# yanconglin/ICP-Flow

Measured on AMD Instinct MI355X. Metric: cluster-pair ICP registrations/sec, higher is better.
Workload: dtype f32

## Files before the change

### icp_flow_amd/build.py

```python
import argparse
import concurrent.futures
import hashlib
import os
import subprocess
import sys

HERE = os.path.dirname(os.path.abspath(__file__))
CSRC = os.path.join(HERE, "csrc")
OBJ = os.path.join(CSRC, "_obj")
OUT = os.path.join(HERE, "libicpflow_hip.so")
SOURCES = ["api.hip", "hist.hip", "nn.hip", "icp.hip", "icp_prep.hip", "icp_plan.hip", "icp_epilogue.hip", "device.hip", "icp_fp32.hip", "pose.hip", "sort.hip", "cluster.hip", "hdbscan.hip", "clusterpcd.hip", "table.hip", "assoc.hip", "frame.hip", "ego.hip", "seqeval.hip", "classeval.hip", "bucketeval.hip", "segeval.hip", "ground.hip", "nnresid.hip", "segresid.hip", "sight.hip",
           "hdbscan_tree.cpp"]
HEADERS = ["common.hpp", "scan.hpp", "kernels.hpp", "kabsch.hpp", "posefuse.hpp", "votekey.hpp", "cluster_util.hpp", "sortdir.hpp", "sortclouds.hpp", "occgrid.hpp", "host.hpp", "carver.hpp", "rowerr.hpp", "clusterpcd_host.hpp", "gridhash.hpp", "nnresid.hpp", "sight.hpp", "icp_instr.hip",
           os.path.join("..", "..", "include", "icpflow_hip.h")]
CFLAGS = ["--offload-arch=gfx950", "-O3", "-std=c++17", "-fPIC", "-ffp-contract=off",
          "-fhip-fp32-correctly-rounded-divide-sqrt", "-Wall", "-Wno-unused-function"]


def hipcc():
    for c in (os.environ.get("HIPCC"), "/opt/rocm/bin/hipcc", "hipcc"):
        if c and (os.path.isabs(c) and os.path.exists(c) or not os.path.isabs(c)):
            return c
    return "hipcc"


def _digest(paths, extra=()):
    h = hashlib.sha256()
    for p in paths:
        h.update(os.path.basename(p).encode())
        with open(p, "rb") as f:
            h.update(f.read())
    for e in extra:
        h.update(str(e).encode())
    return h.hexdigest()


# ... 87 lines not shown
```

### icp_flow_amd/csrc/api.hip

```cpp
#include <stdarg.h>
#include <stdio.h>
#include <stdlib.h>
#include <string.h>

#include "kernels.hpp"
#include "posefuse.hpp"
#include "kabsch.hpp"
#include "host.hpp"

using namespace icpflow;

namespace {

thread_local char g_err[512] = "";

}

namespace icpflow {
int report_error(int code, const char *message)
{
    snprintf(g_err, sizeof(g_err), "%s", message);
    return code;
}

// ... 322 lines not shown
    int dev = -1;
    if (hipGetDevice(&dev) != hipSuccess) { none.ok = false; return none; }
    for (int k = 0; k < kSlots; ++k)
        if (slots[k].used && slots[k].caller == caller && slots[k].s.device == dev) return slots[k].s;
    Slot &sl = slots[next];
    next = (next + 1) % kSlots;
    if (!sl.used || sl.s.device != dev) {
        sl.s.destroy();
        sl.s = SideStream{};
        sl.s.create();
    }
    sl.used = true;
    sl.caller = caller;
    return sl.s;
}

struct JoinGuard {
    hipStream_t s = nullptr;
    hipEvent_t join = nullptr;
    ~JoinGuard() { if (join != nullptr) (void)hipStreamWaitEvent(s, join, 0); }
    void joined() { join = nullptr; }
};

int run_icp_and_select(const float *src, const float *dst, Workspace &w, const uint8_t *swap,
                       const float *init, int B, int N, double thres, int maxIter, double relThr,
                       int stopMode, int invertSwapped, float *Tout, int32_t *iters, const Opts &o, hipStream_t s,
                       bool teamPlanned = false, int part = 0, int32_t *pending = nullptr, bool initSumValid = false)
{
    const GridScratch *search = search_scratch(w, N, o);
    const bool sweepCheck = search != nullptr && search->mode == 3 && o.on(ICPFLOW_OPT_NO_CHECK_SWEEP);
    bool historyPending = false;
    IcpOpts io = o.icp(w.grid.sortX);
    io.help = icp_help_carve(w.ctrl, B, w.helpState, w.helpOut);
    io.splitScratch = w.icpSplit;
    io.teamPlanned = teamPlanned;
    if (sweepCheck && o.arith == ICPFLOW_ARITH_FP64) io.historyPending = &historyPending;
    const bool splittable = sweepCheck && o.arith == ICPFLOW_ARITH_FP64 && stopMode == ICPFLOW_STOP_REFERENCE && w.history != nullptr &&
                            o.on(ICPFLOW_OPT_NO_SPECULATIVE) && maxIter > 1 && maxIter <= kHistIters;
    if (part == 1) {
        *pending = 0;
        if (!splittable) return 0;
        if (icp_teams_wanted(&w.team, io, search, B, N, maxIter, stopMode, w.history)) return 0;
        io.pairActive = nullptr;
    }
    if (part == 2 && pending != nullptr && *pending != 0) {
        historyPending = true;
        if (o.pairActive != nullptr) ICPFLOW_TRY(launch_icp_retally(w.ctrl, w.history, o.pairActive, B, maxIter, relThr, s));
    } else {
        ICPFLOW_TRY(launch_icp(src, dst, w.lenA, w.lenC, swap, init, B, N, thres, maxIter, relThr, stopMode,
                               w.state, w.ctrl, search, w.history, &w.team, io, s));
        if (part == 1) {
            if (!historyPending) return report_errorf(ICPFLOW_E_ARG, "icpflow_register_stage_begin: the ICP launch kept no history");
            *pending = 1;
            return 0;
        }
    }
    if (sweepCheck) {
        PoseSource ps{w.state, w.ctrl, historyPending ? w.history : nullptr, init, B, maxIter};
        const double *initSum = (initSumValid && search->presorted && o.on(ICPFLOW_OPT_NO_CHECK_REUSE)) ? w.scoreAccum : nullptr;
        ICPFLOW_TRY(launch_sweep_check(search, src, dst, w.lenA, w.lenC, swap, B, N, init, nullptr, w.partial, s, &ps, o.pairActive,
                                       initSum));
        ICPFLOW_TRY(launch_select(w.partial, sweep_qblocks(N), w.lenA, w.lenC, swap, init, nullptr, B, invertSwapped,
                                  Tout, s, &ps, iters, initSum, o.pairActive));
        return 0;
    }
    ICPFLOW_TRY(launch_compose(w.state, init, B, w.M, s, w.ctrl, iters));
    {
        ICPFLOW_TRY(launch_scan_check(src, dst, w.lenA, w.lenC, swap, B, N, init, w.M, w.partial, s));
        ICPFLOW_TRY(launch_select(w.partial, scan_qblocks(N, B), w.lenA, w.lenC, swap, init, w.M, B,
                                  invertSwapped, Tout, s));
    }
    return 0;
}

int run_init_pose(const float *src, const float *dst, Workspace &w, const uint8_t *swap, int B,
                  int N, const float *ex, int lx, const float *ey, int ly, const float *ez, int lz,
                  float shift, float *Tout, const Opts &o, hipStream_t s, hipEvent_t joinBefore = nullptr,
                  const PairCountFuse *countFuse = nullptr, bool sideBusy = false, const FrontRoles *roles = nullptr)
{
    const int lens[3] = {lx, ly, lz};
    if (N <= kMaxSortN && o.on(ICPFLOW_OPT_NO_SORTED_VOTE)) {
        bool planned = false;
        ICPFLOW_TRY(launch_hist_vote_sorted(dst, src, w.lenC, w.lenA, B, N, lens, ex, ey, ez, swap, w.zsortC,
                                            w.zsortA, w.bins, w.zckey, w.zcidx, w.voteKey, s, countFuse, sideBusy,
                                            w.grid.pairBox, o.on(ICPFLOW_OPT_NO_VOTE_LIST) ? w.voteWork : nullptr, w.voteWorkCap,
                                            w.pairOrder, &planned, roles));
        if (planned) w.grid.pairOrder = w.pairOrder;
    } else
        ICPFLOW_TRY(launch_hist_vote(dst, src, B, N, N, nullptr, nullptr, lens, ex, ey, ez, swap, w.bins, s));
    if (o.voteBins != nullptr)
        ICPFLOW_TRY(hipMemcpyAsync(o.voteBins, w.bins, (size_t)B * lx * ly * lz * sizeof(uint32_t),
                                   hipMemcpyDeviceToDevice, s));
    if (w.pairTab != nullptr && B <= 700 && N <= kMaxSortN && o.on(ICPFLOW_OPT_NO_SORTED_VOTE)) {
        ICPFLOW_TRY(launch_sweep_pair_table(w.lenA, w.lenC, swap, w.grid.pairOrder, B, N, w.pairTab, s));
        w.grid.pairTab = w.pairTab;
    }
    PeakDecode dec;
    dec.ex = ex; dec.ey = ey; dec.ez = ez; dec.shift = shift; dec.cand = w.cand;
    ICPFLOW_TRY(launch_hist_peaks_u32(w.bins, B, lx, ly, lz, kTopK, kNmsKernel, w.volA, w.volB,
                                      w.peakVotes, w.peakIdx, s, dec));
    if (score_by_sweep(N, joinBefore != nullptr || w.grid.presorted, o)) {
        if (joinBefore != nullptr) {
            ICPFLOW_TRY(hipStreamWaitEvent(s, joinBefore, 0));
        } else if (!w.grid.presorted) {
            ICPFLOW_TRY(launch_sort_clouds_soa(src, dst, w.lenA, w.lenC, swap, B, N, &w.grid, s));
            w.grid.presorted = 1;
            if (o.on(ICPFLOW_OPT_NO_SCORE_PRUNE) && o.on(ICPFLOW_OPT_NO_SCORE_PREBOUND)) {
                ICPFLOW_TRY(launch_occupancy(&w.grid, B, N, s));
                w.grid.occReady = 1;
            }
        }
        if (o.on(ICPFLOW_OPT_NO_SCORE_PRUNE))
            ICPFLOW_TRY(launch_sweep_score_pruned(&w.grid, w.lenA, w.lenC, swap, B, N, w.cand, w.partial, w.scoreAccum, s));
        else
            ICPFLOW_TRY(launch_sweep_score(&w.grid, w.lenA, w.lenC, swap, B, N, w.cand, w.partial, s));
        ICPFLOW_TRY(launch_score_pick(w.partial, sweep_qblocks(N), w.lenA, w.lenC, swap, w.cand, B, Tout, s, w.scoreAccum));
        w.initSumValid = true;
    } else if (o.on(ICPFLOW_OPT_NO_SCORE_PRUNE)) {
        ICPFLOW_TRY(launch_scan_score_pruned(src, dst, w.lenA, w.lenC, swap, B, N, w.cand, w.partial, w.scoreAccum, s, true));
        ICPFLOW_TRY(launch_score_pick(w.partial, score_qblocks(N), w.lenA, w.lenC, swap, w.cand, B, Tout, s));
    } else {
        ICPFLOW_TRY(launch_scan_score(src, dst, w.lenA, w.lenC, swap, B, N, w.cand, w.partial, s));
        ICPFLOW_TRY(launch_score_pick(w.partial, scan_qblocks(N, B), w.lenA, w.lenC, swap, w.cand, B, Tout, s));
    }
    return 0;
}

}

extern "C" {

int icpflow_version(void) { return ICPFLOW_VERSION; }

#ifndef ICPFLOW_SOURCE_HASH
#define ICPFLOW_SOURCE_HASH "unknown"
#endif
static const char g_build_info[] = "ICPFLOW_SOURCE_HASH=" ICPFLOW_SOURCE_HASH;
const char *icpflow_build_info(void) { return g_build_info + sizeof("ICPFLOW_SOURCE_HASH=") - 1; }

const char *icpflow_last_error(void) { return g_err; }
// ... 576 lines not shown
            if (se == hipSuccess) w.grid.occReady = 1;
        }
        if (se == hipSuccess && !countInSort && phase != 1 &&
            icp_teams_wanted(&w.team, o.icp(w.grid.sortX), search, B, N, max_iterations, stop_mode, w.history)) {
            launch_icp_team_plan(&w.team, w.lenA, w.lenC, w.swap, B, N, o.icp(w.grid.sortX), side->stream);
            teamPlanned = true;
        }
        const hipError_t je = hipEventRecord(side->join, side->stream);
        if (je == hipSuccess) { guard.s = s; guard.join = side->join; }
        ICPFLOW_TRY(se);
        ICPFLOW_TRY(je);
        w.grid.presorted = 1;
        join = side->join;
    }
    PairCountFuse fuse{};
    if (countInSort) {
        fuse.swapOut = w.swap;
        fuse.zero0 = w.ctrl; fuse.bytes0 = icp_ctrl_bytes(B);
        fuse.zero1 = w.scoreAccum; fuse.bytes1 = w.accumBytes;
    }
    w.grid.shareCountClean = 1;
    w.grid.sweepTicket = w.ticketScratch;
    const bool sweepScore = score_by_sweep(N, join != nullptr || frontRoles, o);
    if (int r = run_init_pose(d_src, d_dst, w, w.swap, B, N, d_edges_x, len_x, d_edges_y, len_y, d_edges_z,
                              len_z, decode_shift, w.Tinit, o, s, sweepScore ? join : nullptr,
                              countInSort ? &fuse : nullptr, join != nullptr, frontRoles ? &roles : nullptr))
        return r;
    if (join != nullptr && !sweepScore) ICPFLOW_TRY(hipStreamWaitEvent(s, join, 0));
    guard.joined();
    if (phase == 1) {
        carry[0] = w.grid.presorted;
        carry[1] = teamPlanned ? 1 : 0;
        carry[3] = w.initSumValid ? 1 : 0;
        return run_icp_and_select(d_src, d_dst, w, w.swap, w.Tinit, B, N, thres_dist, max_iterations, relative_rmse_thr,
                                  stop_mode, 1, d_T_out, d_iters, o, s, teamPlanned, 1, &carry[2]);
    }
    return run_icp_and_select(d_src, d_dst, w, w.swap, w.Tinit, B, N, thres_dist, max_iterations,
                              relative_rmse_thr, stop_mode, 1, d_T_out, d_iters, o, s, teamPlanned, 0, nullptr, w.initSumValid);
}

int icpflow_hist_icp(const float *d_src, const float *d_dst, int B, int N, const float *d_edges_x,
                     int len_x, const float *d_edges_y, int len_y, const float *d_edges_z, int len_z,
                     float decode_shift, double thres_dist, int max_iterations, double relative_rmse_thr,
                     int stop_mode, float *d_T_out, int32_t *d_iters, void *d_ws, size_t ws_bytes,
                     icpflow_stream_t stream, const icpflow_options_t *opt)
{
    Opts o;
    if (int r = parse_options("icpflow_hist_icp", opt, o)) return r;
    if (int r = check_arith("icpflow_hist_icp", o, max_iterations, stop_mode)) return r;
    if (int r = check_pair_active("icpflow_hist_icp", o, true, max_iterations, stop_mode)) return r;
    if (!d_src || !d_dst || !d_edges_x || !d_edges_y || !d_edges_z || !d_T_out)
        return report_errorf(ICPFLOW_E_ARG, "icpflow_hist_icp: null pointer");
    if (int r = check_batch("icpflow_hist_icp", B, N)) return r;
    if (int r = check_hist_dims("icpflow_hist_icp", len_x, len_y, len_z)) return r;
    if (max_iterations <= 0 || max_iterations > kMaxIterCap)
        return report_errorf(ICPFLOW_E_ARG, "icpflow_hist_icp: max_iterations must be in 1..%d", kMaxIterCap);
    if (stop_mode != ICPFLOW_STOP_REFERENCE && stop_mode != ICPFLOW_STOP_PER_PAIR)
        return report_errorf(ICPFLOW_E_ARG, "icpflow_hist_icp: unknown stop_mode %d", stop_mode);
    const size_t L = (size_t)len_x * len_y * len_z;
    if (L < (size_t)kTopK) return report_errorf(ICPFLOW_E_ARG, "icpflow_hist_icp: fewer than 5 bins");
    Workspace w(d_ws, B, N, L);
// ... 181 lines not shown
```

### icp_flow_amd/csrc/icp.hip

```cpp
#include <atomic>
#include <mutex>

#include "scan.hpp"
#include "sortdir.hpp"
#include "kernels.hpp"
#include "gridhash.hpp"
#include "icp_instr.hip"
#include "kabsch.hpp"

namespace icpflow {

struct IcpParams {
#ifdef ICPFLOW_CERT_STATS
    const float *occHdr;
    const uint32_t *occBits;
#endif
    const float *X;
    const float *Y;
    const int32_t *lenX;
    const int32_t *lenY;
    const uint8_t *swap;
    const float *prePose;
    int N;
    float thr2;
    float relThr;
    int stopMode;
    int maxIter;
    IcpState *state;
    IcpCtrl *ctrl;
    const float4 *gridPts;
    const int32_t *gridStart;
// ... 9 lines not shown
    float *history;
    int B;
    IcpTeam team;
    const float *initR;
    const float *initT;
    int allowReflection;
    int estimateScale;
    const float *initS;
    int halfCu;
    int persistent;
    IcpHelp help;
    int helpOn;
    int redPasses;
    int x0Cache;
    int recCap;
    int shareScans;
    int teamLanes;
    const uint8_t *pairActive;
    int drainAt;
    const int32_t *pairList;
    const int32_t *pairMeta;
    int twoLaunch;
    int32_t *splitScratch;
};


constexpr int kMoments = 18;

__device__ __forceinline__ int state_hash_word(float w, int k)
{
    const unsigned u = (unsigned)__float_as_int(w);
    return (int)__builtin_amdgcn_alignbit(u, u, (unsigned)((5 * k + 3) & 31));
}
constexpr int kRecMaxN = 4096;
#ifndef ICPFLOW_PROBE_MAX
#define ICPFLOW_PROBE_MAX 20
#endif
constexpr int kProbeMax = ICPFLOW_PROBE_MAX;
#ifndef ICPFLOW_PROBE_STEPS
#define ICPFLOW_PROBE_STEPS 8
#endif
constexpr int kProbeSteps = ICPFLOW_PROBE_STEPS;
#ifndef ICPFLOW_PROBE_MAX_LONG
#define ICPFLOW_PROBE_MAX_LONG 32
#endif
#ifndef ICPFLOW_PROBE_STEPS_LONG
// ... 100 lines not shown
#ifdef ICPFLOW_NO_SHARE
    constexpr bool SHARE = false;
#else
    constexpr bool SHARE = SHAREK && TEAM && GRID == 4 && Q == 1;
#endif
    __shared__ int shHdr[SHARE ? NWAVE : 1][4];
    __shared__ int shNext[SHARE ? NWAVE : 1], shDone[SHARE ? NWAVE : 1], shLock[SHARE ? NWAVE : 1];
    __shared__ unsigned int shAcc[SHARE ? NWAVE : 1][3][kWave];
    __shared__ unsigned int shState;
    [[maybe_unused]] const bool helping = HELP && role != 0;
    [[maybe_unused]] HelpPair *hp = nullptr;
    if constexpr (HELP) hp = (p.helpOn && p.help.pair != nullptr) ? p.help.pair + b : nullptr;
    IcpTeam team{};
    if constexpr (TEAM) {
        team.wgPair = p.team.wgPair; team.wgRank = p.team.wgRank; team.teamSize = p.team.teamSize;
        team.arrived = p.team.arrived; team.mom = p.team.mom; team.maxWG = p.team.maxWG;
    }
    const int tid = threadIdx.x;
    const int lane = tid & (kWave - 1);
    const int wave = tid >> 6;
    const int ts = wave % TS;
    const int qg = wave / TS;
    IcpCtrl *ctrl = p.ctrl;
    if (p.pairActive != nullptr && p.history != nullptr && p.pairActive[b] == 0) {
        if (rank == 0 && wave == 0)
            for (int k = itBegin + lane; k < p.maxIter; k += kWave)
                __hip_atomic_fetch_add(&ctrl->tally[k], 1ull, __ATOMIC_RELAXED, __HIP_MEMORY_SCOPE_AGENT);
        if (tid == 0 && rank == 0) {
            IcpState *st0 = p.state + b;
#pragma unroll
            for (int k = 0; k < 9; ++k) st0->R[k] = (k % 4 == 0) ? 1.f : 0.f;
            st0->T[0] = st0->T[1] = st0->T[2] = 0.f;
            st0->rmse = 0.f; st0->s = 1.f; st0->active = 0; st0->iters = 0;
            if constexpr (HELP) {
                if (p.drainAt > 0) __hip_atomic_fetch_add(&ctrl->finished, 1, __ATOMIC_RELAXED, __HIP_MEMORY_SCOPE_AGENT);
            }
        }
        return;
    }
    if (p.stopMode == ICPFLOW_STOP_REFERENCE_ && itBegin > 0 && p.history == nullptr) {
        if (ctrl->done || ctrl->notconv[itBegin - 1] == 0) {
            if (tid == 0 && b == 0) ctrl->done = 1;
            return;
        }
    }
    const bool sw = p.swap != nullptr && p.swap[b] != 0;
    CloudView xc, yc;
    xc.base = (sw ? p.Y : p.X) + (size_t)b * p.N * 4; xc.stride = 4; xc.n = (sw ? p.lenY : p.lenX)[b];
    yc.base = (sw ? p.X : p.Y) + (size_t)b * p.N * 4; yc.stride = 4; yc.n = (sw ? p.lenX : p.lenY)[b];
    PointXf pre;
    pre.kind = p.prePose ? XF_AFFINE : XF_NONE;
    pre.a = p.prePose ? affine_from_pose(p.prePose + (size_t)b * 16) : affine_identity();
    PointXf none;
    none.kind = XF_NONE;
    none.a = affine_identity();

    IcpState *st = p.state + b;
    int active = 1;
    constexpr bool RESUME = BLOCK == 1024 && GRID == 4 && !TEAM && !SCALE && !HELP && LATE && Q == 1 && WIDE;
    const bool resumed = RESUME && itBegin > 0 && p.history != nullptr;
    if (itBegin == 0 || (resumed && itBegin < kRing)) {
        float s0 = (tid < 9 && tid % 4 == 0) ? 1.f : 0.f;
        if (p.initR != nullptr && tid < 12) s0 = tid < 9 ? p.initR[(size_t)b * 9 + tid] : p.initT[(size_t)b * 3 + tid - 9];
        const float scale0 = p.initS != nullptr ? p.initS[b] : 1.f;
        if (itBegin == 0) {
            if (tid < 12) bcast[tid] = s0;
            if (tid == 0) { bcast[12] = 1.f; bcast[13] = 0.f; bcast[14] = 0.f; bcast[15] = scale0; }
        }
        if (tid < 16) ring[tid] = tid < 12 ? s0 : (tid == 14 ? scale0 : 0.f);
        if (tid < kWave) {
            int hash = 0;
#pragma unroll
            for (int k = 0; k < 12; ++k) hash ^= state_hash_word(__shfl(s0, k, kWave), k);
            hash ^= state_hash_word(scale0, 12);
            if (tid == 13) ring[13] = __int_as_float(hash);
// ... 18 lines not shown
                    if (on) ring[(n % kRing) * 16 + w] = w == 13 ? __int_as_float(hw) : hv;
                }
            }
        }
    }
    int itersDone = (itBegin == 0) ? 0 : st->iters;
    if (tid == 0) { probeCnt[0] = 0; probeCnt[1] = 0; probeNext[0] = 0; probeNext[1] = 0; }
    if (SHARE && tid == 0) shState = 0u;
    [[maybe_unused]] int hbSeq = 0;
    [[maybe_unused]] int probePar = 0;

    if (tid == 0) {
        float o0 = 0.f, o1 = 0.f, o2 = 0.f;
        if (xc.n > 0) {
            float rx, ry, rz;
            cloud_load(xc, 0, rx, ry, rz);
            xf_apply(pre, rx, ry, rz, o0, o1, o2);
        }
        bcast[16] = o0; bcast[17] = o1; bcast[18] = o2;
#pragma unroll
        for (int k = 0; k < 9; ++k) preL[k] = pre.a.m[k];
#pragma unroll
        for (int k = 0; k < 3; ++k) preL[9 + k] = pre.a.t[k];
    }
    __syncthreads();

    const int per = NQG * kWave * Q;
    const int ngroups = (xc.n + per - 1) / per;

    int itFirst = itBegin;
    if constexpr (HELP) {
        if (tid == 0) helpSh[0] = 0;
        if (hp == nullptr) __syncthreads();
        if (hp != nullptr && !helping) {
            if (tid == 0) {
                __hip_atomic_store(&hp->passes, (xc.n + BLOCK - 1) / BLOCK, __ATOMIC_RELAXED, __HIP_MEMORY_SCOPE_AGENT);
                __hip_atomic_store(&hp->iter, itBegin + 1, __ATOMIC_RELAXED, __HIP_MEMORY_SCOPE_AGENT);
                __hip_atomic_store(&p.help.owner[blockIdx.x], b + 1, __ATOMIC_RELAXED, __HIP_MEMORY_SCOPE_AGENT);
            }
            __syncthreads();
        }
        if (helping) {
            if (tid == 0) {
                int e = 0;
                const int cur = __hip_atomic_load(&hp->iter, __ATOMIC_RELAXED, __HIP_MEMORY_SCOPE_AGENT);
                if (cur > 0) {
// ... 118 lines not shown
            const int NP16 = (p.N + kChunk - 1) / kChunk * kChunk;
            const int np16 = (yc.n + kChunk - 1) / kChunk * kChunk;
            const float *gx = p.sortYsoa + (size_t)b * 3 * NP16;
            const float *gy = gx + NP16;
            const float *gz = gy + NP16;
            const float4 *ys = p.sortY + (size_t)b * p.N;
            const float4 *xs = p.sortX + (size_t)b * p.N;
            const int axis = sweepAxis;
            float dirX = 0.f, dirY = 0.f;
            if (WIDE && axis >= 3) sort_dir(axis, dirX, dirY);
            unsigned char *dyn = dynLds + (size_t)p.redPasses * (NWAVE * kMoments * sizeof(double));
            float *lx = reinterpret_cast<float *>(dyn), *ly = lx + NP16, *lz = ly + NP16;
            const bool perPass = !TEAM && WIDE && p.redPasses != 0;
            double *redDyn = reinterpret_cast<double *>(dynLds);
            constexpr bool REC = (GRID == 4);
            const int unitsAll = (xc.n + kWave - 1) / kWave;
            const bool dealt = TEAM && G > 1;
            const int myCount = dealt ? (unitsAll > rank ? (unitsAll - rank + G - 1) / G : 0) * kWave : xc.n;
            float4 *rec = reinterpret_cast<float4 *>(dyn + (size_t)NP16 * 12);
            int *recJ = reinterpret_cast<int *>(dyn + (size_t)NP16 * 12 + (size_t)p.recCap * 16);
            const bool recOn = REC && p.recCap > 0 && myCount <= p.recCap;
            float *x0c = reinterpret_cast<float *>(dyn + (size_t)NP16 * 12 + (size_t)p.recCap * 20);
            const bool x0On = recOn && p.x0Cache != 0;
            if (GRID == 4 && it == itFirst) {
                for (int k = tid; k < np16; k += BLOCK) { lx[k] = gx[k]; ly[k] = gy[k]; lz[k] = gz[k]; }
                __syncthreads();
            }
            const float *keyf = (GRID == 4) ? (axis == 0 ? lx : (axis == 1 ? ly : lz))
                                            : (axis == 0 ? gx : (axis == 1 ? gy : gz));
            auto tkey = [&](int j) -> float {
                return (WIDE && axis >= 3) ? sort_key_dir(dirX, dirY, (GRID == 4 ? lx : gx)[j], (GRID == 4 ? ly : gy)[j]) : keyf[j];
            };
            auto pkey = [&](float x, float y, float z) -> float {
                if constexpr (WIDE) return sort_key_of(axis, dirX, dirY, x, y, z);
                else return axis == 0 ? x : (axis == 1 ? y : z);
            };
            auto keySlack = [&](float x, float y, float r) -> float { return WIDE ? sort_key_slack(axis, x, y, r) : 0.f; };
            constexpr int PER = BLOCK * Q;
            const int ngr = (myCount + PER - 1) / PER;
            double fold[5] = {0.0, 0.0, 0.0, 0.0, 0.0};
            bool reuseMoments = false;
            [[maybe_unused]] int helpedPasses = 0;
            if constexpr (HELP) helpedPasses = helping ? 0 : __builtin_amdgcn_readfirstlane(helpSh[0]);
            [[maybe_unused]] bool shareOn = false;
            if constexpr (SHARE) shareOn = recOn && p.shareScans != 0 && yc.n >= kShareMinN;
            [[maybe_unused]] auto unit_query = [&](int gp, int uw, float &ux, float &uy, float &uz) {
                const int li = gp * PER + uw * kWave + lane;
// ... 1409 lines not shown
    } else if (p.gridPts != nullptr) {
        if (p.N <= 256) launch_icp_variant<256, 1, 1, 2>(p, B, itBegin, itEnd, s);
        else if (p.N <= 2048) launch_icp_variant<1024, 1, 1, 2>(p, B, itBegin, itEnd, s);
        else launch_icp_variant<1024, 1, 1, 1>(p, B, itBegin, itEnd, s);
    } else {
        if (p.N <= 256) launch_icp_variant<256, 2, 2, 0>(p, B, itBegin, itEnd, s);
        else if (p.N <= 512) launch_icp_variant<512, 2, 2, 0>(p, B, itBegin, itEnd, s);
        else if (p.N <= 1024) launch_icp_variant<1024, 4, 4, 0>(p, B, itBegin, itEnd, s);
        else launch_icp_variant<1024, 4, 2, 0>(p, B, itBegin, itEnd, s);
    }
    if (timed) profile_stop(prof, s);
}

bool icp_teams_wanted(const IcpTeam *team, const IcpOpts &opts, const GridScratch *grid, int B, int N, int maxIter,
                      int stopMode, const float *history)
{
    const bool speculative = stopMode == ICPFLOW_STOP_REFERENCE_ && history != nullptr && opts.speculative &&
                             maxIter > 1 && maxIter <= kHistIters;
    return opts.arith != ICPFLOW_ARITH_FP32_REFERENCE && team != nullptr && opts.teams && grid != nullptr && grid->mode == 3 &&
           N > 1024 && 2 * B <= device_cus() && B <= 256 && B <= min(icp_team_workgroups(opts), team->maxWG) &&
           (speculative || stopMode == ICPFLOW_STOP_PER_PAIR_);
}

hipError_t launch_icp(const float *X, const float *Y, const int32_t *lenX, const int32_t *lenY,
                      const uint8_t *swap, const float *prePose, int B, int N, double thres,
                      int maxIter, double relThr, int stopMode, IcpState *state, IcpCtrl *ctrl,
                      const GridScratch *grid, float *history, const IcpTeam *team, const IcpOpts &opts,
                      hipStream_t s)
{
    if (opts.arith == ICPFLOW_ARITH_FP32_REFERENCE) {
        if (history == nullptr || opts.fp32Scratch == nullptr || maxIter > kHistIters ||
            stopMode != ICPFLOW_STOP_REFERENCE_)
            return hipErrorInvalidValue;
        return launch_icp_fp32ref(X, Y, lenX, lenY, swap, prePose, B, N, thres, maxIter, relThr, state, ctrl, history,
                                  opts.fp32Scratch, s);
    }
    IcpParams p{};
    bool dirKeys = true;
    p.B = B;
    p.X = X; p.Y = Y; p.lenX = lenX; p.lenY = lenY; p.swap = swap; p.prePose = prePose; p.N = N;
    p.thr2 = (float)(thres * thres);
    p.relThr = (float)relThr;
    p.stopMode = stopMode; p.maxIter = maxIter; p.state = state; p.ctrl = ctrl;
    p.initR = opts.initR; p.initT = opts.initT; p.allowReflection = opts.allowReflection ? 1 : 0;
    p.initS = opts.initS; p.estimateScale = opts.estimateScale ? 1 : 0;
    hipError_t e = hipSuccess;
    bool recWanted = false;
    if (opts.historyPending != nullptr) *opts.historyPending = false;
    if (!opts.ctrlCleared) {
        e = hipMemsetAsync(ctrl, 0, icp_ctrl_bytes(B), s);
        if (e != hipSuccess) return e;
    }
// ... 1 lines not shown
        p.sortX = (const float4 *)grid->sortX; p.sortY = (const float4 *)grid->pts; p.sortAxis = grid->axis;
        dirKeys = N >= kSortDirMinN;
        p.sortYsoa = grid->sortYsoa;
        p.sweepMargin = (float)(1.01 * thres);
#ifdef ICPFLOW_CERT_STATS
        if (grid->occReady) { p.occHdr = grid->occHdr; p.occBits = grid->occBits; }
#endif
        p.sortedRaw = 1;
        recWanted = opts.adaptiveWindows;
    } else if (grid != nullptr && grid->mode == 3) {
        e = launch_sort_clouds(X, Y, lenX, lenY, swap, prePose, B, N, grid, false, nullptr, 0, s);
        if (e != hipSuccess) return e;
        p.sortX = (const float4 *)grid->sortX; p.sortY = (const float4 *)grid->pts; p.sortAxis = grid->axis;
        dirKeys = grid->dirKeys && N >= kSortDirMinN;
        p.sortYsoa = grid->sortYsoa;
        p.sweepMargin = (float)(1.01 * thres);
        recWanted = opts.adaptiveWindows;
    } else if (grid != nullptr) {
        const float invh = (float)(1.0 / (1.01 * thres));
        launch_grid_build(X, Y, lenX, lenY, swap, B, N, invh, grid, s);
        p.gridPts = (const float4 *)grid->pts; p.gridStart = grid->start; p.gridOrigin = grid->origin;
        p.gridH = grid->H; p.gridInvH = invh;
    }
    const int cus = device_cus();
    const bool speculative = stopMode == ICPFLOW_STOP_REFERENCE_ && history != nullptr && opts.speculative &&
                             maxIter > 1 && maxIter <= kHistIters;
    if (icp_teams_wanted(team, opts, grid, B, N, maxIter, stopMode, history)) {
        p.team = *team;
        p.team.maxWG = min(icp_team_workgroups(opts), team->maxWG);
        p.teamLanes = opts.teamsHalfGpu ? 2 : 1;
        if (!opts.teamPlanned) launch_icp_team_plan(team, lenX, lenY, swap, B, N, opts, s);
    }
    if (p.sortY != nullptr) {
        const size_t img = (size_t)((N + kChunk - 1) / kChunk * kChunk) * 12;
        const size_t room = p.team.wgPair != nullptr ? icp_team_room(opts, N) : (size_t)152 * 1024;
        int recCap = 0;
        if (p.team.wgPair != nullptr) {
            if (N <= 12288 && img + 64 * 20 <= room) recCap = (int)((room - img) / 20 / 64 * 64);
            p.shareScans = (recWanted && recCap > 0 && icp_team_shares(opts, N)) ? 1 : 0;
        } else if (N <= kRecMaxN) {
            recCap = N;
        }
        bool x0Cache = recCap > 0 && img + (size_t)recCap * 32 <= room;
        const size_t half = 76 * 1024;
#ifndef ICPFLOW_HALF_CU_MIN_N
#define ICPFLOW_HALF_CU_MIN_N 768
#endif
        const double fillHalf = (double)B / ((double)((B + 2 * cus - 1) / (2 * cus)) * 2 * cus);
        const double fillFull = (double)B / ((double)((B + cus - 1) / cus) * cus);
        const size_t redHalf = N <= kRecMaxN ? (size_t)((N + 511) / 512) * 8 * kMoments * sizeof(double) : 0;
        const size_t redFull = N <= kRecMaxN ? (size_t)((N + 1023) / 1024) * 16 * kMoments * sizeof(double) : 0;
        if (p.team.wgPair == nullptr && B >= 2 * cus && N > ICPFLOW_HALF_CU_MIN_N && redHalf + img + (size_t)recCap * 20 <= half &&
            1.1 * fillHalf > fillFull) {
            p.halfCu = 1;
            x0Cache = redHalf + img + (size_t)recCap * 32 <= half;
        } else if (p.team.wgPair == nullptr) {
            x0Cache = x0Cache && redFull + img + (size_t)recCap * 32 <= room;
        }
        if (recWanted) { p.recCap = recCap; p.x0Cache = x0Cache ? 1 : 0; }
    }
    if (stopMode == ICPFLOW_STOP_REFERENCE_) {
        if (speculative) {
            p.history = history;
            p.pairActive = opts.pairActive;
            p.persistent = opts.persistent ? 1 : 0;
            p.twoLaunch = (opts.twoLaunch && opts.splitScratch != nullptr) ? 1 : 0;
            p.splitScratch = opts.splitScratch;
            p.help = opts.help;
            p.helpOn = (opts.helpers && maxIter <= kHelpMaxEpoch - 2) ? 1 : 0;
            launch_icp_iters(p, dirKeys, B, 0, maxIter, opts.profile, s);
            if (opts.historyPending != nullptr) {
                *opts.historyPending = true;
            } else {
                e = launch_icp_resolve_history(state, ctrl, history, B, maxIter, s);
                if (e != hipSuccess) return e;
            }
        } else {
            for (int it = 0; it < maxIter; ++it) launch_icp_iters(p, dirKeys, B, it, it + 1, opts.profile, s);
        }
    } else {
        p.persistent = opts.persistent ? 1 : 0;
        p.help = opts.help;
        p.helpOn = (opts.helpers && maxIter <= kHelpMaxEpoch - 2) ? 1 : 0;
        launch_icp_iters(p, dirKeys, B, 0, maxIter, opts.profile, s);
    }
    return hipGetLastError();
}

}
```

### icp_flow_amd/csrc/kernels.hpp

```cpp
#pragma once
#include <hip/hip_runtime.h>
#include <atomic>
#include <stddef.h>
#include <stdint.h>

#include "../../include/icpflow_hip.h"

namespace icpflow {

constexpr int ICPFLOW_STOP_REFERENCE_ = ICPFLOW_STOP_REFERENCE;
constexpr int ICPFLOW_STOP_PER_PAIR_ = ICPFLOW_STOP_PER_PAIR;

constexpr int kPartial = 8;
constexpr int kMaxIterCap = 1024;
constexpr int kCand = 6;
constexpr int kTopK = 5;
constexpr int kNmsKernel = 11;

struct IcpState {
    float R[9];
    float T[3];
    float rmse;
    int active;
    int iters;
// ... 169 lines not shown
    int32_t *cursor;
    float *pts;
    float *sortX;
    float *sortYsoa;
    float *sortXsoa;
    int32_t *axis;
    int dirKeys;
    float *ckey;
    int *cidx;
    const float *pairBox;
    const int32_t *pairTab;
    const int32_t *pairOrder;
    float *shareBest;
    int *shareCount;
    int shareCountClean;
    float *occHdr;
    uint32_t *occBits;
    int occReady;
    int32_t *occTot;
    int *sweepTicket;
    int *scoreList;
    int presorted;
};
struct LaunchProfile;
struct IcpOpts {
    int arith = 0;
    bool teams = true;
    bool speculative = true;
    bool adaptiveWindows = true;
    bool persistent = true;
    bool helpers = true;
    IcpHelp help{};
    const float *initR = nullptr;
    const float *initT = nullptr;
    bool allowReflection = false;
    bool estimateScale = false;
    const float *initS = nullptr;
    LaunchProfile *profile = nullptr;
    bool ctrlCleared = false;
    bool *historyPending = nullptr;
    float *fp32Scratch = nullptr;
    bool teamPlanned = false;
    const uint8_t *pairActive = nullptr;
    bool teamsHalfGpu = false;
    bool sharedScans = true;
    bool twoLaunch = false;
    int32_t *splitScratch = nullptr;
};

int device_cus();
void ensure_dynamic_lds(const void *func, int bytes, std::atomic<unsigned long long> *doneMask);
LaunchProfile *profile_create(int capacity, hipError_t *err);
void profile_destroy(LaunchProfile *p);
hipError_t profile_collect(LaunchProfile *p, double *total_ms, int *launches);
bool profile_start(LaunchProfile *p, hipStream_t s);
void profile_stop(LaunchProfile *p, hipStream_t s);

int grid_buckets(int N);
void launch_grid_build(const float *X, const float *Y, const int32_t *lenX, const int32_t *lenY, const uint8_t *swap, int B,
                       int N, float invh, const GridScratch *grid, hipStream_t s);
hipError_t launch_sort_clouds(const float *X, const float *Y, const int32_t *lenX, const int32_t *lenY, const uint8_t *swap,
                              const float *prePose, int B, int N, const GridScratch *grid, bool wantXsoa, const float *boxes,
                              int selfCount, hipStream_t s);
hipError_t launch_sort_clouds_soa(const float *X, const float *Y, const int32_t *lenX, const int32_t *lenY,
                                  const uint8_t *swap, int B, int N, const GridScratch *grid, hipStream_t s, int selfCount = 0);

int icp_team_workgroups(const IcpOpts &opts);
bool icp_team_shares(const IcpOpts &opts, int N);
size_t icp_team_room(const IcpOpts &opts, int N);
void launch_icp_team_plan(const IcpTeam *team, const int32_t *lenX, const int32_t *lenY, const uint8_t *swap, int B, int N,
                          const IcpOpts &opts, hipStream_t s);

bool icp_teams_wanted(const IcpTeam *team, const IcpOpts &opts, const GridScratch *grid, int B, int N, int maxIter,
                      int stopMode, const float *history);
hipError_t launch_icp(const float *X, const float *Y, const int32_t *lenX, const int32_t *lenY,
                      const uint8_t *swap, const float *prePose, int B, int N, double thres,
                      int maxIter, double relThr, int stopMode, IcpState *state, IcpCtrl *ctrl,
                      const GridScratch *grid, float *history, const IcpTeam *team, const IcpOpts &opts,
                      hipStream_t s);
hipError_t launch_icp_fp32ref(const float *X, const float *Y, const int32_t *lenX, const int32_t *lenY,
                              const uint8_t *swap, const float *prePose, int B, int N, double thres, int maxIter,
                              double relThr, IcpState *state, IcpCtrl *ctrl, float *history, float *nnScratch,
                              hipStream_t s);

hipError_t launch_icp_resolve_history(IcpState *state, IcpCtrl *ctrl, const float *history, int B, int maxIter,
                                      hipStream_t s);
hipError_t launch_icp_export(IcpState *state, IcpCtrl *ctrl, int B, int stopMode, float *R,
                             float *T, float *rmse, int32_t *iters, int32_t *converged, hipStream_t s,
                             float *scale = nullptr);
void launch_icp_split(const IcpCtrl *ctrl, const IcpState *state, int B, int maxIter, int32_t *list, int32_t *meta, hipStream_t s);
hipError_t launch_icp_retally(IcpCtrl *ctrl, const float *history, const uint8_t *active, int B, int maxIter, double relThr,
                              hipStream_t s);

hipError_t launch_score_pick(const double *partial, int qblocks, const int32_t *lenA,
                             const int32_t *lenC, const uint8_t *swap, const float *cand, int B,
                             float *Tinit, hipStream_t s, double *initSum = nullptr);
hipError_t launch_compose(const IcpState *state, const float *init, int B, float *M, hipStream_t s,
// ... 62 lines not shown
```

### icp_flow_amd/csrc/pose.hip

```cpp
#include "common.hpp"
#include "kernels.hpp"
#include "posefuse.hpp"

namespace icpflow {

__device__ __forceinline__ double partial_total(const double *partial, int job, int qblocks, int k)
{
    double s = 0.0;
    const double *base = partial + (size_t)job * qblocks * kPartial + k;
    if (qblocks <= 4) {
        double v[4];
#pragma unroll
        for (int u = 0; u < 4; ++u) v[u] = base[(size_t)min(u, qblocks - 1) * kPartial];
#pragma unroll
        for (int u = 0; u < 4; ++u)
            if (u < qblocks) s += v[u];
        return s;
    }
    for (int q0 = 0; q0 < qblocks; q0 += 8) {
        double v[8];
#pragma unroll
        for (int u = 0; u < 8; ++u) v[u] = base[(size_t)min(q0 + u, qblocks - 1) * kPartial];
#pragma unroll
        for (int u = 0; u < 8; ++u)
            if (q0 + u < qblocks) s += v[u];
    }
    return s;
}

__global__ __launch_bounds__(kWave) void score_pick_kernel(const double *__restrict__ partial, int qblocks,
                                                           const int32_t *__restrict__ lenA,
                                                           const int32_t *__restrict__ lenC,
                                                           const uint8_t *__restrict__ swap,
                                                           const float *__restrict__ cand, int B,
                                                           float *__restrict__ Tinit, double *__restrict__ initSum)
{
    const int b = blockIdx.x, lane = threadIdx.x;
    const bool sw = swap != nullptr && swap[b] != 0;
    const float na = (float)(sw ? lenC[b] : lenA[b]);
    const float nc = (float)(sw ? lenA[b] : lenC[b]);
    float mean = 0.f;
    double total = 0.0;
    if (lane < 2 * kCand) {
        total = partial_total(partial, b * 12 + lane, qblocks, 0);
        mean = (float)total / ((lane & 1) ? nc : na);
    }
    int pick = 0;
    float best = 0.f;
    for (int k = 0; k < kCand; ++k) {
        const float sc = fminf(__shfl(mean, 2 * k, kWave), __shfl(mean, 2 * k + 1, kWave));
        if (k == 0 || sc < best) { best = sc; pick = k; }
    }
    if (initSum != nullptr && lane == 2 * pick) initSum[b] = total;
    if (lane < 16) {
        const float *t = cand + ((size_t)b * kCand + pick) * 3;
        float v = (lane % 5 == 0) ? 1.f : 0.f;
        if (lane == 3) v = t[0];
        if (lane == 7) v = t[1];
        if (lane == 11) v = t[2];
        Tinit[(size_t)b * 16 + lane] = v;
    }
}

hipError_t launch_score_pick(const double *partial, int qblocks, const int32_t *lenA,
                             const int32_t *lenC, const uint8_t *swap, const float *cand, int B,
                             float *Tinit, hipStream_t s, double *initSum)
{
    hipLaunchKernelGGL(score_pick_kernel, dim3(B), dim3(kWave), 0, s, partial, qblocks, lenA, lenC, swap, cand, B,
                       Tinit, initSum);
    return hipGetLastError();
}

__global__ void compose_kernel(const IcpState *__restrict__ st, const float *__restrict__ init, int B,
                               float *__restrict__ M, const IcpCtrl *__restrict__ ctrl, int32_t *__restrict__ iters)
{
    const int b = blockIdx.x * blockDim.x + threadIdx.x;
    if (b == 0 && iters != nullptr) *iters = ctrl->error ? -1 : ctrl->iters;
    if (b >= B) return;
    float A[16];
    for (int i = 0; i < 3; ++i) {
        for (int j = 0; j < 3; ++j) A[i * 4 + j] = st[b].R[j * 3 + i];
        A[i * 4 + 3] = st[b].T[i];
    }
    A[12] = A[13] = A[14] = 0.f; A[15] = 1.f;
// ... 340 lines not shown
```

Before: 439,700.

## Fuse candidate score pick into the ICP kernel prologue

Moves the per-pair score-pick step, which chooses the best initial translation candidate, into the first wave of the ICP kernel, so the separate score_pick launch is skipped whenever the speculative grid-mode ICP path qualifies. While wave 0 picks, the other waves preload the sorted target SoA into LDS in the prologue instead of at the first iteration. The goal is to remove one kernel launch and its dependency gap per batch. The cost is a more complex eligibility check that must agree between host and kernel, plus some extra prologue work in the ICP kernel.

```diff
diff --git a/icp_flow_amd/build.py b/icp_flow_amd/build.py
--- a/icp_flow_amd/build.py
+++ b/icp_flow_amd/build.py
@@ -11,7 +11,7 @@
 OUT = os.path.join(HERE, "libicpflow_hip.so")
 SOURCES = ["api.hip", "hist.hip", "nn.hip", "icp.hip", "icp_prep.hip", "icp_plan.hip", "icp_epilogue.hip", "device.hip", "icp_fp32.hip", "pose.hip", "sort.hip", "cluster.hip", "hdbscan.hip", "clusterpcd.hip", "table.hip", "assoc.hip", "frame.hip", "ego.hip", "seqeval.hip", "classeval.hip", "bucketeval.hip", "segeval.hip", "ground.hip", "nnresid.hip", "segresid.hip", "sight.hip",
            "hdbscan_tree.cpp"]
-HEADERS = ["common.hpp", "scan.hpp", "kernels.hpp", "kabsch.hpp", "posefuse.hpp", "votekey.hpp", "cluster_util.hpp", "sortdir.hpp", "sortclouds.hpp", "occgrid.hpp", "host.hpp", "carver.hpp", "rowerr.hpp", "clusterpcd_host.hpp", "gridhash.hpp", "nnresid.hpp", "sight.hpp", "icp_instr.hip",
+HEADERS = ["common.hpp", "scan.hpp", "kernels.hpp", "kabsch.hpp", "posefuse.hpp", "scorepick.hpp", "votekey.hpp", "cluster_util.hpp", "sortdir.hpp", "sortclouds.hpp", "occgrid.hpp", "host.hpp", "carver.hpp", "rowerr.hpp", "clusterpcd_host.hpp", "gridhash.hpp", "nnresid.hpp", "sight.hpp", "icp_instr.hip",
            os.path.join("..", "..", "include", "icpflow_hip.h")]
 CFLAGS = ["--offload-arch=gfx950", "-O3", "-std=c++17", "-fPIC", "-ffp-contract=off",
           "-fhip-fp32-correctly-rounded-divide-sqrt", "-Wall", "-Wno-unused-function"]
diff --git a/icp_flow_amd/csrc/api.hip b/icp_flow_amd/csrc/api.hip
--- a/icp_flow_amd/csrc/api.hip
+++ b/icp_flow_amd/csrc/api.hip
@@ -368,10 +368,29 @@
     void joined() { join = nullptr; }
 };
 
+static bool icp_splittable(const Workspace &w, const GridScratch *search, const Opts &o, int stopMode, int maxIter)
+{
+    const bool sweepCheck = search != nullptr && search->mode == 3 && o.on(ICPFLOW_OPT_NO_CHECK_SWEEP);
+    return sweepCheck && o.arith == ICPFLOW_ARITH_FP64 && stopMode == ICPFLOW_STOP_REFERENCE && w.history != nullptr &&
+           o.on(ICPFLOW_OPT_NO_SPECULATIVE) && maxIter > 1 && maxIter <= kHistIters;
+}
+
+static bool pick_in_icp(Workspace &w, const Opts &o, int B, int N, int maxIter, int stopMode, int phase, bool sweepScore)
+{
+    if (!sweepScore || phase == 2) return false;
+    const GridScratch *search = search_scratch(w, N, o);
+    const IcpOpts io = o.icp(w.grid.sortX);
+    if (phase == 1 && (!icp_splittable(w, search, o, stopMode, maxIter) ||
+                       icp_teams_wanted(&w.team, io, search, B, N, maxIter, stopMode, w.history)))
+        return false;
+    return icp_pick_in_icp(&w.team, io, search, true, B, N, maxIter, stopMode, w.history);
+}
+
 int run_icp_and_select(const float *src, const float *dst, Workspace &w, const uint8_t *swap,
                        const float *init, int B, int N, double thres, int maxIter, double relThr,
                        int stopMode, int invertSwapped, float *Tout, int32_t *iters, const Opts &o, hipStream_t s,
-                       bool teamPlanned = false, int part = 0, int32_t *pending = nullptr, bool initSumValid = false)
+                       bool teamPlanned = false, int part = 0, int32_t *pending = nullptr, bool initSumValid = false,
+                       bool pickInIcp = false)
 {
     const GridScratch *search = search_scratch(w, N, o);
     const bool sweepCheck = search != nullptr && search->mode == 3 && o.on(ICPFLOW_OPT_NO_CHECK_SWEEP);
@@ -381,8 +400,7 @@
     io.splitScratch = w.icpSplit;
     io.teamPlanned = teamPlanned;
     if (sweepCheck && o.arith == ICPFLOW_ARITH_FP64) io.historyPending = &historyPending;
-    const bool splittable = sweepCheck && o.arith == ICPFLOW_ARITH_FP64 && stopMode == ICPFLOW_STOP_REFERENCE && w.history != nullptr &&
-                            o.on(ICPFLOW_OPT_NO_SPECULATIVE) && maxIter > 1 && maxIter <= kHistIters;
+    const bool splittable = icp_splittable(w, search, o, stopMode, maxIter);
     if (part == 1) {
         *pending = 0;
         if (!splittable) return 0;
@@ -393,6 +411,10 @@
         historyPending = true;
         if (o.pairActive != nullptr) ICPFLOW_TRY(launch_icp_retally(w.ctrl, w.history, o.pairActive, B, maxIter, relThr, s));
     } else {
+        if (pickInIcp) {
+            io.pick.partial = w.partial; io.pick.qblocks = sweep_qblocks(N); io.pick.cand = w.cand;
+            io.pick.initSum = w.scoreAccum; io.pick.Tinit = w.Tinit;
+        }
         ICPFLOW_TRY(launch_icp(src, dst, w.lenA, w.lenC, swap, init, B, N, thres, maxIter, relThr, stopMode,
                                w.state, w.ctrl, search, w.history, &w.team, io, s));
         if (part == 1) {
@@ -422,7 +444,8 @@
 int run_init_pose(const float *src, const float *dst, Workspace &w, const uint8_t *swap, int B,
                   int N, const float *ex, int lx, const float *ey, int ly, const float *ez, int lz,
                   float shift, float *Tout, const Opts &o, hipStream_t s, hipEvent_t joinBefore = nullptr,
-                  const PairCountFuse *countFuse = nullptr, bool sideBusy = false, const FrontRoles *roles = nullptr)
+                  const PairCountFuse *countFuse = nullptr, bool sideBusy = false, const FrontRoles *roles = nullptr,
+                  bool pickInIcp = false)
 {
     const int lens[3] = {lx, ly, lz};
     if (N <= kMaxSortN && o.on(ICPFLOW_OPT_NO_SORTED_VOTE)) {
@@ -460,8 +483,11 @@
             ICPFLOW_TRY(launch_sweep_score_pruned(&w.grid, w.lenA, w.lenC, swap, B, N, w.cand, w.partial, w.scoreAccum, s));
         else
             ICPFLOW_TRY(launch_sweep_score(&w.grid, w.lenA, w.lenC, swap, B, N, w.cand, w.partial, s));
-        ICPFLOW_TRY(launch_score_pick(w.partial, sweep_qblocks(N), w.lenA, w.lenC, swap, w.cand, B, Tout, s, w.scoreAccum));
+        if (!pickInIcp)
+            ICPFLOW_TRY(launch_score_pick(w.partial, sweep_qblocks(N), w.lenA, w.lenC, swap, w.cand, B, Tout, s, w.scoreAccum));
         w.initSumValid = true;
+    } else if (pickInIcp) {
+        return report_errorf(ICPFLOW_E_ARG, "hist_icp: the pick was left to the ICP launch, but the scoring did not run as sweeps");
     } else if (o.on(ICPFLOW_OPT_NO_SCORE_PRUNE)) {
         ICPFLOW_TRY(launch_scan_score_pruned(src, dst, w.lenA, w.lenC, swap, B, N, w.cand, w.partial, w.scoreAccum, s, true));
         ICPFLOW_TRY(launch_score_pick(w.partial, score_qblocks(N), w.lenA, w.lenC, swap, w.cand, B, Tout, s));
@@ -1084,9 +1110,10 @@
     w.grid.shareCountClean = 1;
     w.grid.sweepTicket = w.ticketScratch;
     const bool sweepScore = score_by_sweep(N, join != nullptr || frontRoles, o);
+    const bool pickInIcp = pick_in_icp(w, o, B, N, max_iterations, stop_mode, phase, sweepScore);
     if (int r = run_init_pose(d_src, d_dst, w, w.swap, B, N, d_edges_x, len_x, d_edges_y, len_y, d_edges_z,
                               len_z, decode_shift, w.Tinit, o, s, sweepScore ? join : nullptr,
-                              countInSort ? &fuse : nullptr, join != nullptr, frontRoles ? &roles : nullptr))
+                              countInSort ? &fuse : nullptr, join != nullptr, frontRoles ? &roles : nullptr, pickInIcp))
         return r;
     if (join != nullptr && !sweepScore) ICPFLOW_TRY(hipStreamWaitEvent(s, join, 0));
     guard.joined();
@@ -1095,10 +1122,11 @@
         carry[1] = teamPlanned ? 1 : 0;
         carry[3] = w.initSumValid ? 1 : 0;
         return run_icp_and_select(d_src, d_dst, w, w.swap, w.Tinit, B, N, thres_dist, max_iterations, relative_rmse_thr,
-                                  stop_mode, 1, d_T_out, d_iters, o, s, teamPlanned, 1, &carry[2]);
+                                  stop_mode, 1, d_T_out, d_iters, o, s, teamPlanned, 1, &carry[2], false, pickInIcp);
     }
     return run_icp_and_select(d_src, d_dst, w, w.swap, w.Tinit, B, N, thres_dist, max_iterations,
-                              relative_rmse_thr, stop_mode, 1, d_T_out, d_iters, o, s, teamPlanned, 0, nullptr, w.initSumValid);
+                              relative_rmse_thr, stop_mode, 1, d_T_out, d_iters, o, s, teamPlanned, 0, nullptr, w.initSumValid,
+                              pickInIcp);
 }
 
 int icpflow_hist_icp(const float *d_src, const float *d_dst, int B, int N, const float *d_edges_x,
diff --git a/icp_flow_amd/csrc/icp.hip b/icp_flow_amd/csrc/icp.hip
--- a/icp_flow_amd/csrc/icp.hip
+++ b/icp_flow_amd/csrc/icp.hip
@@ -7,6 +7,7 @@
 #include "gridhash.hpp"
 #include "icp_instr.hip"
 #include "kabsch.hpp"
+#include "scorepick.hpp"
 
 namespace icpflow {
 
@@ -62,6 +63,7 @@
     const int32_t *pairMeta;
     int twoLaunch;
     int32_t *splitScratch;
+    IcpPick pick;
 };
 
 
@@ -208,6 +210,13 @@
     const int ts = wave % TS;
     const int qg = wave / TS;
     IcpCtrl *ctrl = p.ctrl;
+    constexpr bool PICK = kPickInIcp && GRID == 4 && !TEAM && !HELP;
+    [[maybe_unused]] float pickW = 0.f;
+    if constexpr (PICK) {
+        if (p.pick.partial != nullptr && wave == 0)
+            pickW = score_pick_wave(p.pick.partial, p.pick.qblocks, p.lenX, p.lenY, p.swap, p.pick.cand, b, lane, p.pick.Tinit,
+                                    p.pick.initSum);
+    }
     if (p.pairActive != nullptr && p.history != nullptr && p.pairActive[b] == 0) {
         if (rank == 0 && wave == 0)
             for (int k = itBegin + lane; k < p.maxIter; k += kWave)
@@ -236,7 +245,15 @@
     yc.base = (sw ? p.X : p.Y) + (size_t)b * p.N * 4; yc.stride = 4; yc.n = (sw ? p.lenX : p.lenY)[b];
     PointXf pre;
     pre.kind = p.prePose ? XF_AFFINE : XF_NONE;
-    pre.a = p.prePose ? affine_from_pose(p.prePose + (size_t)b * 16) : affine_identity();
+    bool picked = false;
+    if constexpr (PICK) picked = p.pick.partial != nullptr;
+    if (picked) {
+        pre.a = affine_identity();
+#pragma unroll
+        for (int k = 0; k < 3; ++k) pre.a.t[k] = __shfl(pickW, 4 * k + 3, kWave);
+    } else {
+        pre.a = p.prePose ? affine_from_pose(p.prePose + (size_t)b * 16) : affine_identity();
+    }
     PointXf none;
     none.kind = XF_NONE;
     none.a = affine_identity();
@@ -301,6 +318,19 @@
         for (int k = 0; k < 9; ++k) preL[k] = pre.a.m[k];
 #pragma unroll
         for (int k = 0; k < 3; ++k) preL[9 + k] = pre.a.t[k];
+    }
+    if constexpr (PICK) {
+        if (!picked || wave != 0) {
+            const int NP16 = (p.N + kChunk - 1) / kChunk * kChunk;
+            const int np16 = (yc.n + kChunk - 1) / kChunk * kChunk;
+            const float *gx = p.sortYsoa + (size_t)b * 3 * NP16;
+            const float *gy = gx + NP16;
+            const float *gz = gy + NP16;
+            float *lx = reinterpret_cast<float *>(dynLds + (size_t)p.redPasses * (NWAVE * kMoments * sizeof(double)));
+            float *ly = lx + NP16, *lz = ly + NP16;
+            const int skip = picked ? kWave : 0;
+            for (int k = tid - skip; k < np16; k += BLOCK - skip) { lx[k] = gx[k]; ly[k] = gy[k]; lz[k] = gz[k]; }
+        }
     }
     __syncthreads();
 
@@ -465,7 +495,7 @@
             const bool recOn = REC && p.recCap > 0 && myCount <= p.recCap;
             float *x0c = reinterpret_cast<float *>(dyn + (size_t)NP16 * 12 + (size_t)p.recCap * 20);
             const bool x0On = recOn && p.x0Cache != 0;
-            if (GRID == 4 && it == itFirst) {
+            if (GRID == 4 && !PICK && it == itFirst) {
                 for (int k = tid; k < np16; k += BLOCK) { lx[k] = gx[k]; ly[k] = gy[k]; lz[k] = gz[k]; }
                 __syncthreads();
             }
@@ -1921,12 +1951,46 @@
            (speculative || stopMode == ICPFLOW_STOP_PER_PAIR_);
 }
 
+#ifndef ICPFLOW_HALF_CU_MIN_N
+#define ICPFLOW_HALF_CU_MIN_N 768
+#endif
+static bool icp_half_cu(int B, int N)
+{
+    const int cus = device_cus();
+    const size_t img = (size_t)((N + kChunk - 1) / kChunk * kChunk) * 12;
+    const size_t recCap = N <= kRecMaxN ? (size_t)N : 0;
+    const size_t half = 76 * 1024;
+    const double fillHalf = (double)B / ((double)((B + 2 * cus - 1) / (2 * cus)) * 2 * cus);
+    const double fillFull = (double)B / ((double)((B + cus - 1) / cus) * cus);
+    const size_t redHalf = N <= kRecMaxN ? (size_t)((N + 511) / 512) * 8 * kMoments * sizeof(double) : 0;
+    return B >= 2 * cus && N > ICPFLOW_HALF_CU_MIN_N && redHalf + img + recCap * 20 <= half && 1.1 * fillHalf > fillFull;
+}
+
+bool icp_pick_in_icp(const IcpTeam *team, const IcpOpts &opts, const GridScratch *grid, bool presorted, int B, int N, int maxIter,
+                     int stopMode, const float *history)
+{
+    if (!kPickInIcp || opts.arith == ICPFLOW_ARITH_FP32_REFERENCE) return false;
+    const bool speculative = stopMode == ICPFLOW_STOP_REFERENCE_ && history != nullptr && opts.speculative &&
+                             maxIter > 1 && maxIter <= kHistIters;
+    if (!speculative) return false;
+    if (grid == nullptr || grid->mode != 3 || !presorted || N > 12288) return false;
+    if (icp_teams_wanted(team, opts, grid, B, N, maxIter, stopMode, history)) return false;
+    const int block = N <= 256 ? 256 : (N <= 512 ? 512 : (N <= 768 ? 768 : (icp_half_cu(B, N) ? 512 : 1024)));
+    const int passes = (N + block - 1) / block;
+    if (opts.persistent && N <= kRecMaxN && passes >= 3 && B > device_cus()) return false;
+    return true;
+}
+
 hipError_t launch_icp(const float *X, const float *Y, const int32_t *lenX, const int32_t *lenY,
                       const uint8_t *swap, const float *prePose, int B, int N, double thres,
                       int maxIter, double relThr, int stopMode, IcpState *state, IcpCtrl *ctrl,
                       const GridScratch *grid, float *history, const IcpTeam *team, const IcpOpts &opts,
                       hipStream_t s)
 {
+    if (opts.pick.partial != nullptr &&
+        (opts.pick.Tinit != prePose || opts.pick.cand == nullptr ||
+         !icp_pick_in_icp(team, opts, grid, grid != nullptr && grid->presorted, B, N, maxIter, stopMode, history)))
+        return hipErrorInvalidValue;
     if (opts.arith == ICPFLOW_ARITH_FP32_REFERENCE) {
         if (history == nullptr || opts.fp32Scratch == nullptr || maxIter > kHistIters ||
             stopMode != ICPFLOW_STOP_REFERENCE_)
@@ -1974,7 +2038,6 @@
         p.gridPts = (const float4 *)grid->pts; p.gridStart = grid->start; p.gridOrigin = grid->origin;
         p.gridH = grid->H; p.gridInvH = invh;
     }
-    const int cus = device_cus();
     const bool speculative = stopMode == ICPFLOW_STOP_REFERENCE_ && history != nullptr && opts.speculative &&
                              maxIter > 1 && maxIter <= kHistIters;
     if (icp_teams_wanted(team, opts, grid, B, N, maxIter, stopMode, history)) {
@@ -1995,15 +2058,9 @@
         }
         bool x0Cache = recCap > 0 && img + (size_t)recCap * 32 <= room;
         const size_t half = 76 * 1024;
-#ifndef ICPFLOW_HALF_CU_MIN_N
-#define ICPFLOW_HALF_CU_MIN_N 768
-#endif
-        const double fillHalf = (double)B / ((double)((B + 2 * cus - 1) / (2 * cus)) * 2 * cus);
-        const double fillFull = (double)B / ((double)((B + cus - 1) / cus) * cus);
         const size_t redHalf = N <= kRecMaxN ? (size_t)((N + 511) / 512) * 8 * kMoments * sizeof(double) : 0;
         const size_t redFull = N <= kRecMaxN ? (size_t)((N + 1023) / 1024) * 16 * kMoments * sizeof(double) : 0;
-        if (p.team.wgPair == nullptr && B >= 2 * cus && N > ICPFLOW_HALF_CU_MIN_N && redHalf + img + (size_t)recCap * 20 <= half &&
-            1.1 * fillHalf > fillFull) {
+        if (p.team.wgPair == nullptr && icp_half_cu(B, N)) {
             p.halfCu = 1;
             x0Cache = redHalf + img + (size_t)recCap * 32 <= half;
         } else if (p.team.wgPair == nullptr) {
@@ -2020,6 +2077,7 @@
             p.splitScratch = opts.splitScratch;
             p.help = opts.help;
             p.helpOn = (opts.helpers && maxIter <= kHelpMaxEpoch - 2) ? 1 : 0;
+            p.pick = opts.pick;
             launch_icp_iters(p, dirKeys, B, 0, maxIter, opts.profile, s);
             if (opts.historyPending != nullptr) {
                 *opts.historyPending = true;
diff --git a/icp_flow_amd/csrc/kernels.hpp b/icp_flow_amd/csrc/kernels.hpp
--- a/icp_flow_amd/csrc/kernels.hpp
+++ b/icp_flow_amd/csrc/kernels.hpp
@@ -215,6 +215,18 @@
     int *scoreList;
     int presorted;
 };
+#ifdef ICPFLOW_NO_PICK_IN_ICP
+constexpr bool kPickInIcp = false;
+#else
+constexpr bool kPickInIcp = true;
+#endif
+struct IcpPick {
+    const double *partial = nullptr;
+    int qblocks = 0;
+    const float *cand = nullptr;
+    double *initSum = nullptr;
+    float *Tinit = nullptr;
+};
 struct LaunchProfile;
 struct IcpOpts {
     int arith = 0;
@@ -239,6 +251,7 @@
     bool sharedScans = true;
     bool twoLaunch = false;
     int32_t *splitScratch = nullptr;
+    IcpPick pick{};
 };
 
 int device_cus();
@@ -266,6 +279,8 @@
 
 bool icp_teams_wanted(const IcpTeam *team, const IcpOpts &opts, const GridScratch *grid, int B, int N, int maxIter,
                       int stopMode, const float *history);
+bool icp_pick_in_icp(const IcpTeam *team, const IcpOpts &opts, const GridScratch *grid, bool presorted, int B, int N, int maxIter,
+                     int stopMode, const float *history);
 hipError_t launch_icp(const float *X, const float *Y, const int32_t *lenX, const int32_t *lenY,
                       const uint8_t *swap, const float *prePose, int B, int N, double thres,
                       int maxIter, double relThr, int stopMode, IcpState *state, IcpCtrl *ctrl,
diff --git a/icp_flow_amd/csrc/pose.hip b/icp_flow_amd/csrc/pose.hip
--- a/icp_flow_amd/csrc/pose.hip
+++ b/icp_flow_amd/csrc/pose.hip
@@ -1,32 +1,9 @@
 #include "common.hpp"
 #include "kernels.hpp"
 #include "posefuse.hpp"
+#include "scorepick.hpp"
 
 namespace icpflow {
-
-__device__ __forceinline__ double partial_total(const double *partial, int job, int qblocks, int k)
-{
-    double s = 0.0;
-    const double *base = partial + (size_t)job * qblocks * kPartial + k;
-    if (qblocks <= 4) {
-        double v[4];
-#pragma unroll
-        for (int u = 0; u < 4; ++u) v[u] = base[(size_t)min(u, qblocks - 1) * kPartial];
-#pragma unroll
-        for (int u = 0; u < 4; ++u)
-            if (u < qblocks) s += v[u];
-        return s;
-    }
-    for (int q0 = 0; q0 < qblocks; q0 += 8) {
-        double v[8];
-#pragma unroll
-        for (int u = 0; u < 8; ++u) v[u] = base[(size_t)min(q0 + u, qblocks - 1) * kPartial];
-#pragma unroll
-        for (int u = 0; u < 8; ++u)
-            if (q0 + u < qblocks) s += v[u];
-    }
-    return s;
-}
 
 __global__ __launch_bounds__(kWave) void score_pick_kernel(const double *__restrict__ partial, int qblocks,
                                                            const int32_t *__restrict__ lenA,
@@ -35,31 +12,7 @@
                                                            const float *__restrict__ cand, int B,
                                                            float *__restrict__ Tinit, double *__restrict__ initSum)
 {
-    const int b = blockIdx.x, lane = threadIdx.x;
-    const bool sw = swap != nullptr && swap[b] != 0;
-    const float na = (float)(sw ? lenC[b] : lenA[b]);
-    const float nc = (float)(sw ? lenA[b] : lenC[b]);
-    float mean = 0.f;
-    double total = 0.0;
-    if (lane < 2 * kCand) {
-        total = partial_total(partial, b * 12 + lane, qblocks, 0);
-        mean = (float)total / ((lane & 1) ? nc : na);
-    }
-    int pick = 0;
-    float best = 0.f;
-    for (int k = 0; k < kCand; ++k) {
-        const float sc = fminf(__shfl(mean, 2 * k, kWave), __shfl(mean, 2 * k + 1, kWave));
-        if (k == 0 || sc < best) { best = sc; pick = k; }
-    }
-    if (initSum != nullptr && lane == 2 * pick) initSum[b] = total;
-    if (lane < 16) {
-        const float *t = cand + ((size_t)b * kCand + pick) * 3;
-        float v = (lane % 5 == 0) ? 1.f : 0.f;
-        if (lane == 3) v = t[0];
-        if (lane == 7) v = t[1];
-        if (lane == 11) v = t[2];
-        Tinit[(size_t)b * 16 + lane] = v;
-    }
+    (void)score_pick_wave(partial, qblocks, lenA, lenC, swap, cand, blockIdx.x, threadIdx.x, Tinit, initSum);
 }
 
 hipError_t launch_score_pick(const double *partial, int qblocks, const int32_t *lenA,
diff --git a/icp_flow_amd/csrc/scorepick.hpp b/icp_flow_amd/csrc/scorepick.hpp
--- /dev/null
+++ b/icp_flow_amd/csrc/scorepick.hpp
@@ -0,0 +1,63 @@
+#pragma once
+#include "common.hpp"
+#include "kernels.hpp"
+
+namespace icpflow {
+
+__device__ __forceinline__ double partial_total(const double *partial, int job, int qblocks, int k)
+{
+    double s = 0.0;
+    const double *base = partial + (size_t)job * qblocks * kPartial + k;
+    if (qblocks <= 4) {
+        double v[4];
+#pragma unroll
+        for (int u = 0; u < 4; ++u) v[u] = base[(size_t)min(u, qblocks - 1) * kPartial];
+#pragma unroll
+        for (int u = 0; u < 4; ++u)
+            if (u < qblocks) s += v[u];
+        return s;
+    }
+    for (int q0 = 0; q0 < qblocks; q0 += 8) {
+        double v[8];
+#pragma unroll
+        for (int u = 0; u < 8; ++u) v[u] = base[(size_t)min(q0 + u, qblocks - 1) * kPartial];
+#pragma unroll
+        for (int u = 0; u < 8; ++u)
+            if (q0 + u < qblocks) s += v[u];
+    }
+    return s;
+}
+
+__device__ __forceinline__ float score_pick_wave(const double *partial, int qblocks, const int32_t *lenA, const int32_t *lenC,
+                                                 const uint8_t *swap, const float *cand, int b, int lane, float *Tinit,
+                                                 double *initSum)
+{
+    const bool sw = swap != nullptr && swap[b] != 0;
+    const float na = (float)(sw ? lenC[b] : lenA[b]);
+    const float nc = (float)(sw ? lenA[b] : lenC[b]);
+    float mean = 0.f;
+    double total = 0.0;
+    if (lane < 2 * kCand) {
+        total = partial_total(partial, b * 12 + lane, qblocks, 0);
+        mean = (float)total / ((lane & 1) ? nc : na);
+    }
+    int pick = 0;
+    float best = 0.f;
+    for (int k = 0; k < kCand; ++k) {
+        const float sc = fminf(__shfl(mean, 2 * k, kWave), __shfl(mean, 2 * k + 1, kWave));
+        if (k == 0 || sc < best) { best = sc; pick = k; }
+    }
+    if (initSum != nullptr && lane == 2 * pick) initSum[b] = total;
+    float v = 0.f;
+    if (lane < 16) {
+        const float *t = cand + ((size_t)b * kCand + pick) * 3;
+        v = (lane % 5 == 0) ? 1.f : 0.f;
+        if (lane == 3) v = t[0];
+        if (lane == 7) v = t[1];
+        if (lane == 11) v = t[2];
+        Tinit[(size_t)b * 16 + lane] = v;
+    }
+    return v;
+}
+
+}
```

New measurement: 444,400 (median of 6 runs). 1.01x the previous value.
